# beehive-lab/GPULlama3.java

Hardware: AMD Instinct MI355X
Metric: tg128 tok/s (llama-bench), Llama-3-8B Q8_0 (higher is better)
Workload: dtype i8; 1 GPU; Llama-3-8B-random Q8_0 random-weight GGUF-layout model, tg128 at depth 0 (one step = 128 decode tokens, logits D2H inside the timed region); parallelism=single GPU, ranks=1, ctx=648

## Files before the change

### gpullama3.java_amd/csrc/gl3_api.hip

```cpp
#include <chrono>
#include <cstdio>
#include <cstdlib>
#include <cstring>
#include <vector>

#include "gl3_ctx.h"
#include "gl3_batch_plan.h"
#include "gl3_decode_kernels.h"
#include "gl3_rowlane_kernels.h"
#include "gl3_veclane_kernels.h"
#include "gl3_moe_kernels.h"
#include "gl3_kv_copy.h"

using namespace gl3;

static std::string g_create_err;

static double now_ms() {
    return std::chrono::duration<double, std::milli>(std::chrono::steady_clock::now().time_since_epoch()).count();
}


static size_t matvec_smem(int pro, int epi, const Q8Mat& w) {
    const int nm = epi == EPI_SWIGLU ? 2 : 1;
// ... 318 lines not shown
    if (!ctx->use_rccl) return GL3_OK;
    pr.begin(GL3_K_COLLECTIVE, 0);
    const int32_t r = gl3_all_gather(ctx, which, (size_t)count_per_rank);
    if (r != GL3_OK) return r;
    pr.end();
    return GL3_OK;
}

enum { ATT_LONG = 0, ATT_SHORT = 1, ATT_MID = 2 };
static int attn_mode(const gl3_ctx* ctx, int pos) {
    return (ctx->fused_attn_ok && pos < AF_MAXN) ? ATT_SHORT : pos < ctx->attn_mid ? ATT_MID : ATT_LONG;
}

static void launch_attention(gl3_ctx* ctx, int l, int which , int amode = ATT_LONG) {
    const gl3_model_desc& d = ctx->d;
    gl3_layer& L = ctx->layers[l];
    const size_t kv_layer = (size_t)d.ctx * ctx->kv_dim_l;
    const int kvmul = d.n_heads / d.n_kv_heads;
    AttnArgs aa{};
    aa.qkv = ctx->qkv; aa.kcache = ctx->kcache + l * kv_layer; aa.vcache = ctx->vcache + l * kv_layer;
    aa.rope_cr = ctx->rope_cr; aa.rope_ci = ctx->rope_ci; aa.qnorm = L.qnorm; aa.knorm = L.knorm; aa.bq = L.bq; aa.bk = L.bk; aa.bv = L.bv;
    aa.dyn = ctx->dyn_cur; aa.att = ctx->att; aa.xb = ctx->xb + (size_t)d.tp_rank * ctx->q_dim_l;
    aa.n_heads = ctx->heads_l; aa.n_kv_heads = ctx->kv_heads_l;
    aa.hs = d.head_size; aa.q_dim = ctx->q_dim_l; aa.kv_dim = ctx->kv_dim_l; aa.ctx = d.ctx;
    aa.eps = d.rms_eps; aa.arch = ctx->rope_arch; aa.att_mul = ctx->att_mul;
    const size_t sm1 = ((size_t)kvmul * d.head_size + (size_t)ATT_TT * (d.head_size + 4) + d.head_size) * 4;
    const int pv_rows = d.ctx < PV_ROWS ? d.ctx : PV_ROWS;
    aa.win = ctx->attn_win;
    aa.att_stride = (d.ctx + 3) & ~3;
    aa.att_t = ctx->att_t; aa.tmax = ctx->att_tmax; aa.sums = ctx->att_sums;
    aa.tp = tp_rec(ctx, l, TR_ATTN);
    const size_t sm2 = ((size_t)ctx->attn_win + (size_t)pv_rows * PV_COLS) * 4;
    if (which == 0 && amode == ATT_SHORT && ctx->fused_attn_ok) {
        attn_head_dispatch(d.head_size, [&](auto kern) { hipLaunchKernelGGL(kern, dim3(ctx->heads_l), dim3(256), attn_head_smem(d.head_size), ctx->stream, aa); });
        return;
    }
    static const bool scores_loop = env_flag("GL3_ATTN_SCORES_LOOP", true);
    if (which != 2 && amode == ATT_LONG && scores_loop && kvmul <= 4 && (d.head_size == 128 || d.head_size == 64)) {
        const dim3 sg(ctx->n_tsplit < SCL_WGS ? ctx->n_tsplit : SCL_WGS, ctx->kv_heads_l), sb(64 * (kvmul + SCL_LOADERS));
        const size_t sml = ((size_t)kvmul * d.head_size + 2 * (size_t)ATT_TT * (d.head_size + 4) + 2 * d.head_size) * 4;
        if (d.head_size == 128) hipLaunchKernelGGL(attn_scores_loop_kernel<128>, sg, sb, sml, ctx->stream, aa, ctx->n_tsplit);
        else hipLaunchKernelGGL(attn_scores_loop_kernel<64>, sg, sb, sml, ctx->stream, aa, ctx->n_tsplit);
    }
    else if (which != 2) hipLaunchKernelGGL(attn_scores_kernel, dim3(ctx->n_tsplit, ctx->kv_heads_l), dim3(64 * kvmul), sm1, ctx->stream, aa);
    if (which != 1 && amode == ATT_LONG) {
        const int exp_rows = (d.ctx + EXP_ROW - 1) / EXP_ROW;
        hipLaunchKernelGGL(attn_exp_kernel, dim3(exp_rows < EXP_GRID_MAX ? exp_rows : EXP_GRID_MAX, ctx->heads_l), dim3(256), 0, ctx->stream, aa, ctx->n_tsplit);
        hipLaunchKernelGGL(attn_sum_kernel, dim3(ctx->heads_l), dim3(256), attn_sum_smem(), ctx->stream, aa);
        hipLaunchKernelGGL(attn_pv_kernel, dim3(ctx->kv_heads_l * attn_pv_hq(kvmul) * (d.head_size / PV_COLS16)), dim3(64 * PV_WAVES), attn_pv_smem(), ctx->stream, aa);
    } else if (which != 1)
        hipLaunchKernelGGL(attn_softmax_pv_kernel, dim3(ctx->heads_l * (d.head_size / PV_COLS)), dim3(256), sm2, ctx->stream, aa);
}

static int32_t enqueue_decode(gl3_ctx* ctx, bool want_logits, gl3_kernel_times* kt, int amode) {
    const gl3_model_desc& d = ctx->d;
    hipStream_t s = ctx->stream;
    Prof pr{ctx, kt};
    const int rank = d.tp_rank;
    const bool q8 = ctx->emb.fmt == GL3_TYPE_Q8_0;
    int32_t r;
    Gl3Range step_range("gl3 decode step");

    pr.begin(GL3_K_OTHER, (uint64_t)d.dim / 32 * 34);
    const int fold = ctx->tp_fold, fmask = fold ? ctx->tp_fold_mask : 0, L_ = d.n_layers;
    uint32_t* vl_step = fold ? reinterpret_cast<uint32_t*>(ctx->arena.base + GL3_ARENA_STEP) : (uint32_t*)nullptr;
    if (ctx->emb.fmt == GL3_TYPE_Q8_0)
        hipLaunchKernelGGL(embed_q8t_kernel, dim3(1), dim3(256), 0, s, ctx->emb.w, ctx->emb.ng, d.dim, ctx->dyn_cur, ctx->x, ctx->emb_scale,
// ... 236 lines not shown
    const size_t kvn = ctx->kv_seq_stride * ctx->n_seqs;
    TRY(dmalloc(ctx, &ctx->kcache, kvn));
    TRY(dmalloc(ctx, &ctx->vcache, kvn + (size_t)PVT * ctx->kv_dim_l));
    TRYHIP(hipMemset(ctx->kcache, 0, kvn * 4));
    TRYHIP(hipMemset(ctx->vcache, 0, (kvn + (size_t)PVT * ctx->kv_dim_l) * 4));
    if (ctx->n_seqs > 1) TRY(dmalloc(ctx, &ctx->kv_copy_dst, ctx->n_seqs));
    TRY(dmalloc(ctx, &ctx->xn, d.dim));
    TRY(dmalloc(ctx, &ctx->qkv, ctx->q_dim_l + 2 * ctx->kv_dim_l));
    if (ctx->use_rccl) {
        if (tp > GL3_MAX_TP) return bail(GL3_E_UNSUPPORTED, "tp_size above 16");
        TRY(gl3_tp_arena_alloc(ctx));
        ctx->x = (float*)(ctx->arena.base + ctx->arena.off[GB_X]); ctx->xb = (float*)(ctx->arena.base + ctx->arena.off[GB_XB]);
        ctx->hb = (float*)(ctx->arena.base + ctx->arena.off[GB_HB]); ctx->logits = (float*)(ctx->arena.base + ctx->arena.off[GB_LOGITS]);
    } else {
        TRY(dmalloc(ctx, &ctx->x, d.dim));
        TRY(dmalloc(ctx, &ctx->xb, ctx->q_dim));
        TRY(dmalloc(ctx, &ctx->hb, d.hidden));
        TRY(dmalloc(ctx, &ctx->logits, d.vocab));
    }
    TRY(dmalloc(ctx, &ctx->att, (size_t)ctx->heads_l * ((d.ctx + 3) & ~3)));
    TRY(dmalloc(ctx, &ctx->att_t, attn_att_t_floats(ctx->kv_heads_l, d.n_heads / d.n_kv_heads, (d.ctx + 3) & ~3)));
    TRYHIP(hipMemset(ctx->att_t, 0, attn_att_t_floats(ctx->kv_heads_l, d.n_heads / d.n_kv_heads, (d.ctx + 3) & ~3) * 4));
    TRY(dmalloc(ctx, &ctx->att_tmax, (size_t)ctx->heads_l * ctx->n_tsplit));
    TRY(dmalloc(ctx, &ctx->att_sums, (size_t)ctx->heads_l));
    if (moe) TRY(moe_build_slots(ctx));
    TRYHIP((allow_big_lds<PRO_RMS, EPI_STORE>()));
    TRYHIP((allow_big_lds<PRO_QUANT, EPI_RESID>()));
    TRYHIP((allow_big_lds<PRO_RMS, EPI_SWIGLU>()));
    {
        ctx->fused_attn_ok = d.head_size % 4 == 0 && attn_head_smem(d.head_size) <= 150 * 1024 && !env_flag("GL3_NO_FUSED_ATTN", false);
        if (ctx->fused_attn_ok) {
            hipError_t ae = hipSuccess;
            attn_head_dispatch(d.head_size, [&](auto kern) { ae = hipFuncSetAttribute((const void*)kern, hipFuncAttributeMaxDynamicSharedMemorySize, 160 * 1024 - 256); });
            TRYHIP(ae);
        }
    }
    TRYHIP(hipFuncSetAttribute((const void*)matvec_q8t_kernel<PRO_QUANT, EPI_RESID, true, 8>, hipFuncAttributeMaxDynamicSharedMemorySize, 160 * 1024 - 256));
    TRYHIP(hipFuncSetAttribute((const void*)matvec_q8t_kernel<PRO_QUANT, EPI_RESID, true, 8, false, false, true>, hipFuncAttributeMaxDynamicSharedMemorySize, 160 * 1024 - 256));
    TRYHIP(hipFuncSetAttribute((const void*)matvec_q8t_kernel<PRO_QUANT, EPI_RESID, true, 8, false, true, true>, hipFuncAttributeMaxDynamicSharedMemorySize, 160 * 1024 - 256));
#define GL3_RL_LDS(...) TRYHIP(hipFuncSetAttribute((const void*)matvec_rl_kernel<__VA_ARGS__>, hipFuncAttributeMaxDynamicSharedMemorySize, 160 * 1024 - 256))
    GL3_RL_LDS(WT_F16, EPI_STORE); GL3_RL_LDS(WT_F16, EPI_RESID); GL3_RL_LDS(WT_F16, EPI_SWIGLU);
    GL3_RL_LDS(WT_Q4_0, EPI_STORE); GL3_RL_LDS(WT_Q4_0, EPI_RESID); GL3_RL_LDS(WT_Q4_0, EPI_SWIGLU);
#undef GL3_RL_LDS
    TRYHIP(hipFuncSetAttribute((const void*)rmsnorm_f32_kernel, hipFuncAttributeMaxDynamicSharedMemorySize, 160 * 1024 - 256));
    TRYHIP(hipFuncSetAttribute((const void*)attn_scores_kernel, hipFuncAttributeMaxDynamicSharedMemorySize, 128 * 1024));
    TRYHIP(hipFuncSetAttribute((const void*)attn_scores_loop_kernel<128>, hipFuncAttributeMaxDynamicSharedMemorySize, 128 * 1024));
    TRYHIP(hipFuncSetAttribute((const void*)attn_scores_loop_kernel<64>, hipFuncAttributeMaxDynamicSharedMemorySize, 128 * 1024));
    TRYHIP(hipFuncSetAttribute((const void*)attn_softmax_pv_kernel, hipFuncAttributeMaxDynamicSharedMemorySize, 150 * 1024));
    TRYHIP(hipFuncSetAttribute((const void*)attn_sum_kernel, hipFuncAttributeMaxDynamicSharedMemorySize, (int)attn_sum_smem()));
    TRYHIP(hipFuncSetAttribute((const void*)attn_pv_kernel, hipFuncAttributeMaxDynamicSharedMemorySize, (int)attn_pv_smem()));
    {
        const char* wv = getenv("GL3_ATTN_WINDOW");
        int wmax = wv && *wv ? atoi(wv) : 16384;
        if (wmax < PV_ROWS || wmax % PV_ROWS != 0 || wmax > 16384) return bail(GL3_E_ARG, "GL3_ATTN_WINDOW must be a multiple of 1024 between 1024 and 16384");
        ctx->attn_win = d.ctx <= wmax ? ((d.ctx + 3) & ~3) : wmax;
        const char* mv = getenv("GL3_ATTN_MID");
        ctx->attn_mid = mv && *mv ? atoi(mv) : 768;
    }
    TRY(dmalloc(ctx, &ctx->dyn, GL3_DYN_INTS));
    ctx->dyn_cur = ctx->dyn;
    TRY(dmalloc(ctx, &ctx->argmax, 2 + 2 * AMX_WGS));
    TRYHIP(hipMemset(ctx->argmax, 0, (2 + 2 * AMX_WGS) * sizeof(int)));
    if (d.flags & GL3_FLAG_LAYER_TAPS) TRY(dmalloc(ctx, &ctx->taps, (size_t)d.n_layers * d.dim));
    TRYHIP(hipHostMalloc((void**)&ctx->h_dyn, GL3_DYN_INTS * sizeof(int)));
    TRYHIP(hipHostMalloc((void**)&ctx->h_logits, (size_t)d.vocab * 4));
    TRYHIP(hipHostMalloc((void**)&ctx->h_argmax, sizeof(int)));
// ... 877 lines not shown
```

### gpullama3.java_amd/csrc/gl3_decode_kernels.h

```cpp
#pragma once
#include <hip/hip_runtime.h>
#include <stdint.h>

#include "gl3_seqsum.h"

namespace gl3 {

constexpr int TILE_BYTES = 2176;
constexpr int MV_AUX = 4;
__host__ __device__ constexpr int mv_threads(int npw) { return 64 * (npw + MV_AUX); }

enum { PRO_RMS = 0, PRO_QUANT = 1 };
enum { EPI_STORE = 0, EPI_RESID = 1, EPI_SWIGLU = 2 };
__host__ __device__ constexpr int mv_ch(int epi) { return epi == EPI_SWIGLU ? 4 : 8; }
__host__ __device__ constexpr int mv_seg_groups(int npw, int epi) { return npw * mv_ch(epi); }

typedef float v4f __attribute__((ext_vector_type(4)));

#ifdef GL3_MV_TIMING
__device__ long long gl3_mv_stamp[32];
#define ATT_STAMP(i) do { if (blockIdx.x == 0 && threadIdx.x == 0) gl3_mv_stamp[i] = wall_clock64(); } while (0)
#define MV_STAMP(i, cond) do { if (blockIdx.x == 0 && (cond)) gl3_mv_stamp[i] = clock64(); } while (0)
#define PV_T(...) __VA_ARGS__
constexpr int MV_WG_STAMPS = 1024;
__device__ unsigned long long gl3_mv_wg_stamp[MV_WG_STAMPS][8];
#define MV_WG_TIME(v) v = (unsigned long long)wall_clock64()
#define MV_WG_PUT(s, v, cond) do { if (blockIdx.x < MV_WG_STAMPS && blockIdx.y == 0 && (cond)) atomicMax(&gl3_mv_wg_stamp[blockIdx.x][s], v); } while (0)
#else
#define PV_T(...)
#define MV_STAMP(i, cond)
#define MV_WG_TIME(v)
#define MV_WG_PUT(s, v, cond)
#define ATT_STAMP(i)
#endif

constexpr int TPF_MAX_PEERS = 15;
struct TpWait {
    const uint32_t* flags;
    const uint32_t* step;
    uint32_t* err;
    int mul, add, tp, me;
    unsigned spin_limit;
};
struct TpPush {
    uint32_t* ticket;
    const uint32_t* step;
    int mul, add, npeers;
    long delta[TPF_MAX_PEERS];
    uint32_t* flag[TPF_MAX_PEERS];
};
struct TpRec { TpWait w; TpPush p; };

__device__ __forceinline__ void tp_wait(const TpWait& w) {
    const uint32_t need = (__hip_atomic_load(w.step, __ATOMIC_RELAXED, __HIP_MEMORY_SCOPE_AGENT) - 1u) * (uint32_t)w.mul + (uint32_t)w.add;
// ... 217 lines not shown
    if (t < 2) sync_w[t] = 0;

    if (wave < MV_PRODUCERS) {
        const int nt = (a.ng - wave + MV_PRODUCERS - 1) / MV_PRODUCERS;
        uint16_t sc[NM][CH];
        int4 lo[NM][CH], hi[NM][CH];
        auto issue = [&](int strip, int i0) {
#pragma unroll
            for (int u = 0; u < CH; ++u) {
                if (i0 + u < nt) {
                    const int g = wave + (i0 + u) * MV_PRODUCERS;
#pragma unroll
                    for (int m = 0; m < NM; ++m) {
                        const uint8_t* p = (m == 0 ? a.w : a.w2) + (size_t)strip * strip_bytes + (size_t)g * TILE_BYTES;
                        sc[m][u] = ld2<NT>(p + 2 * lane);
                        lo[m][u] = ld16<NT>(p + 128 + 16 * lane);
                        hi[m][u] = ld16<NT>(p + 1152 + 16 * lane);
                    }
                }
            }
        };
        auto compute = [&](int i0, float* pb) {
#pragma unroll
            for (int u = 0; u < CH; ++u) {
                if (i0 + u < nt) {
                    const int g = wave + (i0 + u) * MV_PRODUCERS;
                    const int xb = 4 * g + (lane >> 4);
                    const int4 xlo = *reinterpret_cast<const int4*>(xq + 32 * xb);
                    const int4 xhi = *reinterpret_cast<const int4*>(xq + 32 * xb + 16);
                    const float xsc = xs[xb];
#pragma unroll
                    for (int m = 0; m < NM; ++m) {
                        const int isum = dot32(lo[m][u], hi[m][u], xlo, xhi);
                        pb[(size_t)m * a.ng * 64 + g * 64 + lane] = (float)isum * (h2f(sc[m][u]) * xsc);
                    }
                }
            }
        };
        int strip = blockIdx.x;
        __syncthreads();
        if (strip < a.nstrips) issue(strip, 0);
        while (__hip_atomic_load(&sync_w[1], __ATOMIC_RELAXED, __HIP_MEMORY_SCOPE_WORKGROUP) == 0) __builtin_amdgcn_s_sleep(2);
        __builtin_amdgcn_fence(__ATOMIC_ACQUIRE, "workgroup");
        MV_STAMP(3, t == 0);
        int it = 0;
        for (; strip < a.nstrips; strip += gridDim.x, ++it) {
            float* pb = pbuf + (size_t)(it & 1) * NM * a.ng * 64;
            for (int i0 = 0; i0 < nt; i0 += CH) {
                if (it != 0 || i0 != 0) issue(strip, i0);
                compute(i0, pb);
                if (SEGS) {
                    MV_STAMP(4 + 2 * it, t == 0 && it < 4 && i0 + CH >= nt);
                    MV_WG_TIME(wg_t1);
                    lds_barrier();
                }
            }
            if (SEGS) {
                for (int b = (nt + CH - 1) / CH; b < nbatch; ++b) lds_barrier();
            } else {
                MV_STAMP(4 + 2 * it, t == 0 && it < 4);
                MV_WG_TIME(wg_t1);
                __syncthreads();
            }
            MV_STAMP(5 + 2 * it, t == 0 && it < 4);
        }
        MV_WG_PUT(0, wg_t0, t == 0); MV_WG_PUT(1, wg_t1, lane == 0);
        return;
// ... 53 lines not shown
        *reinterpret_cast<int4*>(xq + 32 * b) = z;
        *reinterpret_cast<int4*>(xq + 32 * b + 16) = z;
    }
    if (nquads <= NXV * 256) {
#pragma unroll
        for (int i = 0; i < NXV; ++i) {
            const int qd = ta + 256 * i;
            if (qd < nquads) {
                float4 v = xv[i];
                if (PRO == PRO_RMS) {
                    const float4 w = nwv[i];
                    v.x = w.x * (scale * v.x); v.y = w.y * (scale * v.y); v.z = w.z * (scale * v.z); v.w = w.w * (scale * v.w);
                }
                quantize_quad(v, qd, xq, xs);
            }
        }
    } else {
        for (int qd = ta; qd < nquads; qd += 256) {
            float4 v = *reinterpret_cast<const float4*>(a.x + 4 * qd);
            if (PRO == PRO_RMS) {
                const float4 w = *reinterpret_cast<const float4*>(a.norm_w + 4 * qd);
                v.x = w.x * (scale * v.x); v.y = w.y * (scale * v.y); v.z = w.z * (scale * v.z); v.w = w.w * (scale * v.w);
            }
            quantize_quad(v, qd, xq, xs);
        }
    }
    aux_sync();
    if (ta == 0) __hip_atomic_store(&sync_w[1], 1, __ATOMIC_RELEASE, __HIP_MEMORY_SCOPE_WORKGROUP);
    if (wave != MV_PRODUCERS) return;

    int it = 0;
    for (int strip = blockIdx.x; strip < a.nstrips; strip += gridDim.x, ++it) {
        const float* pb = pbuf + (size_t)(it & 1) * NM * a.ng * 64;
        v4f acc[NM];
#pragma unroll
        for (int m = 0; m < NM; ++m) acc[m] = (v4f){0.f, 0.f, 0.f, 0.f};
        for (int b = 0; b < nbatch; ++b) {
            if (SEGS) lds_barrier(); else __syncthreads();
            MV_STAMP(16 + 2 * it, lane == 0 && it < 4 && b == nbatch - 1);
            MV_WG_TIME(wg_t1);
            int g = b * SEG;
            const int ge = SEGS ? min(g + SEG, a.ng) : a.ng;
            for (; g + 8 <= ge; g += 8) {
                float av[NM][8];
#pragma unroll
                for (int m = 0; m < NM; ++m)
#pragma unroll
                    for (int u = 0; u < 8; ++u) av[m][u] = pb[(size_t)m * a.ng * 64 + (g + u) * 64 + lane];
#pragma unroll
                for (int u = 0; u < 8; ++u)
#pragma unroll
                    for (int m = 0; m < NM; ++m) acc[m] = __builtin_amdgcn_mfma_f32_16x16x4f32(av[m][u], 1.0f, acc[m], 0, 0, 0);
            }
            for (; g < ge; ++g)
#pragma unroll
                for (int m = 0; m < NM; ++m)
                    acc[m] = __builtin_amdgcn_mfma_f32_16x16x4f32(pb[(size_t)m * a.ng * 64 + g * 64 + lane], 1.0f, acc[m], 0, 0, 0);
        }
        MV_STAMP(17 + 2 * it, lane == 0 && it < 4);
        MV_WG_TIME(wg_t2);
        if ((lane & 15) < 4) {
            const int r = lane & 3;
            const int row = strip * 16 + 4 * (lane >> 4) + r;
            if (row < a.rows) {
                const float v0 = r == 0 ? acc[0][0] : r == 1 ? acc[0][1] : r == 2 ? acc[0][2] : acc[0][3];
                float res;
                if (EPI == EPI_STORE) res = v0 * a.out_scale;
                if (EPI == EPI_RESID) res = a.resid_in ? a.resid_in[row] + v0 * a.out_scale : v0 * a.out_scale;
                if (EPI == EPI_SWIGLU) {
                    const float v1 = r == 0 ? acc[NM - 1][0] : r == 1 ? acc[NM - 1][1] : r == 2 ? acc[NM - 1][2] : acc[NM - 1][3];
                    const float gte = v0 / (float)(1.0 + exp(-(double)v0));
                    res = gte * v1;
                }
                a.out[row] = res;
                if (TPF) tp_push_store(a.tp->p, a.out + row, res);
            }
        }
        PV_T(asm volatile("s_waitcnt vmcnt(0)" ::: "memory");)
        MV_WG_TIME(wg_t0);
        MV_WG_PUT(2, wg_t1, lane == 0); MV_WG_PUT(3, wg_t2, lane == 0); MV_WG_PUT(4, wg_t0, lane == 0);
    }
    if (TPF && a.tp->p.npeers) tp_publish(a.tp->p, gridDim.x);
}

static __global__ __launch_bounds__(256) void embed_q8t_kernel(const uint8_t* __restrict__ emb, int ng, int dim,
                                                         const int* __restrict__ dyn, float* __restrict__ x, float emb_scale,
                                                         const TpRec* tp = nullptr, uint32_t* step = nullptr) {
    if (step) {
        const uint32_t s = *step;
        __syncthreads();
        if (threadIdx.x == 0) *step = s + 1;
        if (tp) {
            TpWait w = tp->w;
            const uint32_t need = s * (uint32_t)w.mul;
            const int lane = threadIdx.x & 63;
            const bool mine = lane < w.tp && lane != w.me;
            unsigned spins = 0;
            for (;;) {
                const bool ok = !mine || (int32_t)(__hip_atomic_load(w.flags + (mine ? lane : 0), __ATOMIC_RELAXED, __HIP_MEMORY_SCOPE_SYSTEM) - need) >= 0;
                if (__builtin_amdgcn_ballot_w64(!ok) == 0) break;
                __builtin_amdgcn_s_sleep(8);
                if (++spins > w.spin_limit) { if (lane == 0) __hip_atomic_store(w.err, 1u, __ATOMIC_RELAXED, __HIP_MEMORY_SCOPE_SYSTEM); break; }
            }
// ... 25 lines not shown
    const float* bv;
    const int* dyn;
    float* att;
    float* xb;
    int n_heads, n_kv_heads, hs, q_dim, kv_dim, ctx;
    float eps;
    int arch;
    const int* seqv;
    const int* posv;
    size_t seq_stride;
    int qkv_stride, xb_stride;
    float att_mul;
    int win;
    int att_stride;
    float* att_t;
    float* tmax;
    float* sums;
    int group;
    uint8_t* xq_out; float* xs_out; int xq_slots;
    const TpRec* tp;
};

__device__ __forceinline__ void rope_head(float* v, int hs, const float* cr, const float* ci, int arch, int t0, int nthreads) {
    const int half = hs >> 1;
    for (int i = t0; i < half; i += nthreads) {
        const float fcr = cr[i], fci = ci[i];
        const int i0 = arch == 0 ? 2 * i : i, i1 = arch == 0 ? 2 * i + 1 : i + half;
        const float v0 = v[i0], v1 = v[i1];
        v[i0] = v0 * fcr - v1 * fci;
        v[i1] = v0 * fci + v1 * fcr;
    }
}

__device__ __forceinline__ void head_rmsnorm_wave(float* v, const float* __restrict__ w, int hs, float eps, int lane) {
    float ss = seq_sum_lds<true>(v, hs);
    ss /= (float)hs;
    ss += eps;
    ss = (float)(1.0 / sqrt((double)ss));
    for (int i = lane; i < hs; i += 64) v[i] = w[i] * (ss * v[i]);
}

constexpr int ATT_TT = 64;

static __global__ void attn_scores_kernel(const AttnArgs a) {
    extern __shared__ __attribute__((aligned(16))) float sm[];
    const int hs = a.hs, kvmul = a.n_heads / a.n_kv_heads, half = hs >> 1;
    float* q_s = sm;
    float* kt = q_s + kvmul * hs;
    float* cr_s = kt + ATT_TT * (hs + 4);
    float* ci_s = cr_s + half;
    const int t = threadIdx.x, nthr = blockDim.x;
    const int sp = blockIdx.x, kvh = blockIdx.y;
    const int pos = a.dyn[1];
    const int t0 = sp * ATT_TT;
    if (t0 > pos) return;
    const int t1 = min(pos + 1, t0 + ATT_TT);
    const bool owns_pos = (t1 == pos + 1);
    const int pitch = hs + 4;
    float* krow = kt + (pos - t0) * pitch;
    const int q4 = hs >> 2;
    const int nrows_cache = owns_pos ? (t1 - 1 - t0) : (t1 - t0);
    const int nk4 = nrows_cache * q4;
    constexpr int KMAX = 16;
    float4 kreg[KMAX];
    const int per = (nk4 + nthr - 1) / nthr;
#pragma unroll
    for (int u = 0; u < KMAX; ++u) {
        kreg[u] = make_float4(0.f, 0.f, 0.f, 0.f);
        if (u < per) {
            const int i = min(t + u * nthr, nk4 - 1);
            kreg[u] = *reinterpret_cast<const float4*>(a.kcache + (size_t)(t0 + i / q4) * a.kv_dim + kvh * hs + 4 * (i % q4));
// ... 166 lines not shown
#define SCL_USE(Q_, K_) do { _Pragma("unroll") for (int u = 0; u < 4; ++u) { \
            score = score + mul_f32_scalar(Q_[u].x, K_[u].x); score = score + mul_f32_scalar(Q_[u].y, K_[u].y); \
            score = score + mul_f32_scalar(Q_[u].z, K_[u].z); score = score + mul_f32_scalar(Q_[u].w, K_[u].w); } } while (0)
        SCL_RD(qa, ka, 0);
#pragma unroll
        for (int g = 0; g < HS / 16; g += 2) {
            SCL_RD(qb, kb, 4 * (g + 1));
            __builtin_amdgcn_sched_barrier(0);
            SCL_USE(qa, ka);
            __builtin_amdgcn_sched_barrier(0);
            if (g + 2 < HS / 16) SCL_RD(qa, ka, 4 * (g + 2));
            __builtin_amdgcn_sched_barrier(0);
            SCL_USE(qb, kb);
            __builtin_amdgcn_sched_barrier(0);
        }
#undef SCL_RD
#undef SCL_USE
        float my_score = -INFINITY;
        if (t0 + r < t1) {
            my_score = a.att_mul != 0.f ? score * a.att_mul : score / sqrt_hs;
            a.att[(size_t)(kvh * kvmul + hq) * a.att_stride + t0 + r] = my_score;
        }
        const float m = wave_max(my_score);
        if (r == 0) a.tmax[(size_t)(kvh * kvmul + hq) * n_tiles_max + sp] = m;
    }
    PV_T(if (blockIdx.x == 0 && blockIdx.y == 0 && t == 0) { gl3_mv_stamp[5] = cbw_; gl3_mv_stamp[6] = clock64() - cts_; gl3_mv_stamp[7] = cnt; })
}

constexpr int AF_MAXN = 128;
__host__ __device__ inline size_t attn_head_smem(int hs, int group = 1) {
    return ((size_t)group * hs + (size_t)AF_MAXN * (hs + 4) + (size_t)AF_MAXN * hs + (size_t)group * AF_MAXN + hs + 16) * 4;
}

template <int HS>
static __global__ __launch_bounds__(256, 1) void attn_head_kernel(const AttnArgs a) {
    extern __shared__ __attribute__((aligned(16))) float sm[];
    const int hs = HS > 0 ? HS : a.hs, kvmul = a.n_heads / a.n_kv_heads, half = hs >> 1, pitch = hs + 4, q4 = hs >> 2;
    const int q4sh = (q4 & (q4 - 1)) == 0 ? __ffs(q4) - 1 : -1;
    auto row_of = [&](int i) { return q4sh >= 0 ? i >> q4sh : i / q4; };
    auto col_of = [&](int i, int row) { return q4sh >= 0 ? i & (q4 - 1) : i - row * q4; };
    const int G = a.group > 1 ? a.group : 1;
    float* q_s = sm;
    float* kt = q_s + G * hs;
    float* vt = kt + AF_MAXN * pitch;
    float* e_s = vt + AF_MAXN * hs;
    float* cr_s = e_s + G * AF_MAXN;
    float* ci_s = cr_s + half;
    float* red = ci_s + half;
    const int t = threadIdx.x, lane = t & 63, wave = t >> 6;
    const int h0 = blockIdx.x * G, kvh = h0 / kvmul;
    const bool owner = (h0 % kvmul) == 0;
    const int bt = blockIdx.y;
    const int pos = a.seqv ? a.posv[bt] : a.dyn[1], n = pos + 1;
    const size_t kvoff = a.seqv ? (size_t)a.seqv[bt] * a.seq_stride : 0;
    const float* qkv = a.qkv + (size_t)bt * a.qkv_stride;
    float* kcache = a.kcache + kvoff;
    float* vcache = a.vcache + kvoff;
    ATT_STAMP(0);
    const int nk4 = pos * q4;
    constexpr int KMAX = 16;
    float4 kreg[KMAX], vreg[KMAX];
    const bool in_regs = nk4 <= KMAX * 256;
    const int per = in_regs ? (nk4 + 255) >> 8 : 0;
#pragma unroll
    for (int u = 0; u < KMAX; ++u) {
        kreg[u] = make_float4(0.f, 0.f, 0.f, 0.f);
        vreg[u] = make_float4(0.f, 0.f, 0.f, 0.f);
        if (u < per) {
            const int i = min(t + u * 256, nk4 - 1), ri = row_of(i);
            const size_t off = (size_t)ri * a.kv_dim + kvh * hs + 4 * col_of(i, ri);
            kreg[u] = *reinterpret_cast<const float4*>(kcache + off);
            vreg[u] = *reinterpret_cast<const float4*>(vcache + off);
        }
    }
    for (int i = t; i < G * hs; i += 256) q_s[i] = a.bq ? qkv[h0 * hs + i] + a.bq[h0 * hs + i] : qkv[h0 * hs + i];
    for (int i = t; i < half; i += 256) { cr_s[i] = a.rope_cr[(size_t)pos * half + i]; ci_s[i] = a.rope_ci[(size_t)pos * half + i]; }
    float* krow = kt + pos * pitch;
    for (int i = t; i < hs; i += 256) {
        krow[i] = a.bk ? qkv[a.q_dim + kvh * hs + i] + a.bk[kvh * hs + i] : qkv[a.q_dim + kvh * hs + i];
        vt[pos * hs + i] = a.bv ? qkv[a.q_dim + a.kv_dim + kvh * hs + i] + a.bv[kvh * hs + i] : qkv[a.q_dim + a.kv_dim + kvh * hs + i];
    }
    if (in_regs) {
#pragma unroll
        for (int u = 0; u < KMAX; ++u) {
            const int i = t + u * 256;
            if (i < nk4) {
                const int ri = row_of(i), ci = col_of(i, ri);
                *reinterpret_cast<float4*>(kt + ri * pitch + 4 * ci) = kreg[u];
                *reinterpret_cast<float4*>(vt + ri * hs + 4 * ci) = vreg[u];
            }
        }
    } else {
        for (int i = t; i < nk4; i += 256) {
            const int ri = row_of(i), ci = col_of(i, ri);
            const size_t off = (size_t)ri * a.kv_dim + kvh * hs + 4 * ci;
            *reinterpret_cast<float4*>(kt + ri * pitch + 4 * ci) = *reinterpret_cast<const float4*>(kcache + off);
            *reinterpret_cast<float4*>(vt + ri * hs + 4 * ci) = *reinterpret_cast<const float4*>(vcache + off);
        }
    }
    __syncthreads();
    ATT_STAMP(1);
    if (a.arch == 1) {
        for (int vec = wave; vec <= G; vec += 4)
            head_rmsnorm_wave(vec < G ? q_s + vec * hs : krow, vec < G ? a.qnorm : a.knorm, hs, a.eps, lane);
        __syncthreads();
    }
    for (int g = 0; g < G; ++g) rope_head(q_s + g * hs, hs, cr_s, ci_s, a.arch, t, 256);
    rope_head(krow, hs, cr_s, ci_s, a.arch, t, 256);
    __syncthreads();
    if (owner) {
        for (int i = t; i < hs; i += 256) {
            kcache[(size_t)pos * a.kv_dim + kvh * hs + i] = krow[i];
            vcache[(size_t)pos * a.kv_dim + kvh * hs + i] = vt[pos * hs + i];
        }
    }
    ATT_STAMP(2);
    const float sqrt_hs = (float)sqrt((double)hs);
    float sc = -INFINITY;
    for (int idx = t; idx < G * n; idx += 256) {
        const int g = idx / n, tt = idx - g * n;
        const float* q = q_s + g * hs;
        const float* kk = kt + tt * pitch;
        float score = 0.f;
        float4 qv = *reinterpret_cast<const float4*>(q), kv = *reinterpret_cast<const float4*>(kk);
        for (int j = 4; j < hs; j += 4) {
            const float4 qn = *reinterpret_cast<const float4*>(q + j), kn = *reinterpret_cast<const float4*>(kk + j);
            score = score + qv.x * kv.x; score = score + qv.y * kv.y; score = score + qv.z * kv.z; score = score + qv.w * kv.w;
            qv = qn; kv = kn;
        }
        score = score + qv.x * kv.x; score = score + qv.y * kv.y; score = score + qv.z * kv.z; score = score + qv.w * kv.w;
        sc = a.att_mul != 0.f ? score * a.att_mul : score / sqrt_hs;
        if (G > 1) e_s[g * AF_MAXN + tt] = sc;
    }
    ATT_STAMP(3);
    if (G == 1) {
        {
            const float wm = wave_max(t < n ? sc : -INFINITY);
            if (lane == 0) red[wave] = wm;
        }
        __syncthreads();
        const float mx = fmaxf(fmaxf(red[0], red[1]), fmaxf(red[2], red[3]));
        float ex = 0.f;
        if (t < n) { ex = (float)exp((double)(sc - mx)); e_s[t] = ex; }
        __syncthreads();
        ATT_STAMP(4);
        if (wave == 0) { const float sum = seq_sum_lds_ring(e_s, n); if (lane == 0) red[4] = sum; }
        __syncthreads();
        if (t < n) e_s[t] = ex / red[4];
        __syncthreads();
    } else {
        __syncthreads();
        for (int g = wave; g < G; g += 4) {
            float* e = e_s + g * AF_MAXN;
            const float s0 = lane < n ? e[lane] : -INFINITY, s1 = lane + 64 < n ? e[lane + 64] : -INFINITY;
            const float mx = wave_max(fmaxf(s0, s1));
            const float e0 = lane < n ? (float)exp((double)(s0 - mx)) : 0.f, e1 = lane + 64 < n ? (float)exp((double)(s1 - mx)) : 0.f;
            if (lane < n) e[lane] = e0;
            if (lane + 64 < n) e[lane + 64] = e1;
            __builtin_amdgcn_fence(__ATOMIC_RELEASE, "workgroup");
            __builtin_amdgcn_wave_barrier();
            __builtin_amdgcn_fence(__ATOMIC_ACQUIRE, "workgroup");
            const float sum = seq_sum_lds_ring(e, n);
            __builtin_amdgcn_wave_barrier();
            if (lane < n) e[lane] = e0 / sum;
            if (lane + 64 < n) e[lane + 64] = e1 / sum;
        }
        __syncthreads();
    }
    ATT_STAMP(5);
    for (int idx = t; idx < G * hs; idx += 256) {
        const int g = idx / hs, j = idx - g * hs;
        const float* e = e_s + g * AF_MAXN;
        const float* vj = vt + j;
        float acc = 0.f;
        int tt = 0;
        const int NG = n >> 2;
        if (NG >= 3) {
            float4 ea, eb, ec;
            float a0, a1, a2, a3, b0, b1, b2, b3, c0, c1, c2, c3;
#define PV_LD(G_, E_, V0_, V1_, V2_, V3_) do { const int r_ = 4 * min((G_), NG - 1); E_ = *reinterpret_cast<const float4*>(e + r_); \
            const float* vr_ = vj + r_ * hs; V0_ = vr_[0]; V1_ = vr_[hs]; V2_ = vr_[2 * hs]; V3_ = vr_[3 * hs]; } while (0)
#define PV_ACC(E_, V0_, V1_, V2_, V3_) do { acc = mul_f32_scalar(E_.x, V0_) + acc; acc = mul_f32_scalar(E_.y, V1_) + acc; \
            acc = mul_f32_scalar(E_.z, V2_) + acc; acc = mul_f32_scalar(E_.w, V3_) + acc; } while (0)
            PV_LD(0, ea, a0, a1, a2, a3); PV_LD(1, eb, b0, b1, b2, b3); PV_LD(2, ec, c0, c1, c2, c3);
            int gq = 0;
            for (; gq + 3 <= NG; gq += 3) {
                PV_ACC(ea, a0, a1, a2, a3); PV_LD(gq + 3, ea, a0, a1, a2, a3); __builtin_amdgcn_sched_barrier(0);
                PV_ACC(eb, b0, b1, b2, b3); PV_LD(gq + 4, eb, b0, b1, b2, b3); __builtin_amdgcn_sched_barrier(0);
                PV_ACC(ec, c0, c1, c2, c3); PV_LD(gq + 5, ec, c0, c1, c2, c3); __builtin_amdgcn_sched_barrier(0);
            }
            if (gq < NG) { PV_ACC(ea, a0, a1, a2, a3); ++gq; }
            if (gq < NG) { PV_ACC(eb, b0, b1, b2, b3); ++gq; }
#undef PV_ACC
#undef PV_LD
            tt = 4 * NG;
        }
        for (; tt < n; ++tt) acc = e[tt] * vj[tt * hs] + acc;
        if (a.xq_out) {
            float am = fabsf(acc);
            am = fmaxf(am, __builtin_bit_cast(float, __builtin_amdgcn_update_dpp(0, __builtin_bit_cast(int, am), 0xB1, 0xf, 0xf, false)));
            am = fmaxf(am, __builtin_bit_cast(float, __builtin_amdgcn_update_dpp(0, __builtin_bit_cast(int, am), 0x4E, 0xf, 0xf, false)));
            am = fmaxf(am, __builtin_bit_cast(float, __builtin_amdgcn_update_dpp(0, __builtin_bit_cast(int, am), 0x141, 0xf, 0xf, false)));
            am = fmaxf(am, __builtin_bit_cast(float, __builtin_amdgcn_update_dpp(0, __builtin_bit_cast(int, am), 0x140, 0xf, 0xf, false)));
            am = fmaxf(am, __shfl_xor(am, 16, 64));
            const float qs = am / 127.0f;
            const float ainv = qs != 0.f ? 1.0f / qs : 0.f;
            const float sv = acc * ainv;
            const int q0 = (int)(sv + copysignf(0.5f, sv)) & 0xFF;
            const int q1 = __builtin_amdgcn_update_dpp(0, q0, 0x55, 0xf, 0xf, false);
            const int q2 = __builtin_amdgcn_update_dpp(0, q0, 0xAA, 0xf, 0xf, false);
            const int q3 = __builtin_amdgcn_update_dpp(0, q0, 0xFF, 0xf, 0xf, false);
            const int el = (h0 + g) * hs + j;
            if ((lane & 3) == 0)
                *reinterpret_cast<uint32_t*>(a.xq_out + bdq_offset(el >> 2, bt, a.xq_slots)) = (uint32_t)q0 | ((uint32_t)q1 << 8) | ((uint32_t)q2 << 16) | ((uint32_t)q3 << 24);
            if ((lane & 31) == 0) a.xs_out[bds_offset(el >> 5, bt, a.xq_slots)] = (float)(_Float16)qs;
        } else {
            float* o = a.xb + (size_t)bt * a.xb_stride + (size_t)(h0 + g) * hs + j;
            *o = acc;
            if (a.tp) tp_push_store(a.tp->p, o, acc);
        }
    }
    ATT_STAMP(6);
    if (a.tp) tp_publish(a.tp->p, gridDim.x * gridDim.y * 4);
}

template <typename F>
static inline void attn_head_dispatch(int hs, F&& f) {
    if (hs == 128) f(attn_head_kernel<128>);
    else if (hs == 64) f(attn_head_kernel<64>);
    else f(attn_head_kernel<0>);
}

constexpr int PV_COLS = 16;
constexpr int PV_ROWS = 1024;

static __global__ __launch_bounds__(256) void attn_softmax_pv_kernel(const AttnArgs a) {
    extern __shared__ __attribute__((aligned(16))) float e_s[];
    const int hs = a.hs, kvmul = a.n_heads / a.n_kv_heads;
    const int nj = hs / PV_COLS;
    const int h = blockIdx.x / nj, j0 = (blockIdx.x % nj) * PV_COLS;
    const int t = threadIdx.x, lane = t & 63, wave = t >> 6, kvh = h / kvmul;
    const int n = a.dyn[1] + 1;
    float* vbuf = e_s + a.win;
    const float* vbase = a.vcache + kvh * hs + j0;
    constexpr int SU = PV_ROWS * 4 / 256;
    float4 sreg[SU];
#pragma unroll
    for (int u = 0; u < SU; ++u) sreg[u] = make_float4(0.f, 0.f, 0.f, 0.f);
    auto stage_issue = [&](int r0, int nr) {
#pragma unroll
        for (int u = 0; u < SU; ++u) {
            if (64 * u < nr) {
                const int row = min((t >> 2) + 64 * u, nr - 1);
                sreg[u] = *reinterpret_cast<const float4*>(vbase + (size_t)(r0 + row) * a.kv_dim + 4 * (t & 3));
            }
        }
    };
    auto stage_commit = [&](int nr) {
#pragma unroll
        for (int u = 0; u < SU; ++u)
            if ((t >> 2) + 64 * u < nr) *reinterpret_cast<float4*>(vbuf + 4 * (t + 256 * u)) = sreg[u];
    };
    __shared__ float red_s[8];
// ... 358 lines not shown
```

Baseline: 477.7 tok/s.

## Split fused short-context attention head kernel across value-column slices

The fused per-head attention kernel now launches a second grid dimension that splits the head's value columns into slices (2 for head size 128, 4 for 64). Each block recomputes the scores but loads and multiplies only its slice of V, so the decode attention stage gets more workgroups. The kernel also prefetches q/k/v/rope and norm weights into registers, defers V staging until after the softmax, and swaps some syncthreads for LDS-only barriers. The cost is redundant QK and softmax work in every slice, and the K-cache row is written only by slice zero.

```diff
diff --git a/gpullama3.java_amd/csrc/gl3_api.hip b/gpullama3.java_amd/csrc/gl3_api.hip
--- a/gpullama3.java_amd/csrc/gl3_api.hip
+++ b/gpullama3.java_amd/csrc/gl3_api.hip
@@ -374,7 +374,7 @@
     aa.tp = tp_rec(ctx, l, TR_ATTN);
     const size_t sm2 = ((size_t)ctx->attn_win + (size_t)pv_rows * PV_COLS) * 4;
     if (which == 0 && amode == ATT_SHORT && ctx->fused_attn_ok) {
-        attn_head_dispatch(d.head_size, [&](auto kern) { hipLaunchKernelGGL(kern, dim3(ctx->heads_l), dim3(256), attn_head_smem(d.head_size), ctx->stream, aa); });
+        attn_head_cs_dispatch(d.head_size, [&](auto kern, int cs, size_t smem) { hipLaunchKernelGGL(kern, dim3(ctx->heads_l, cs), dim3(256), smem, ctx->stream, aa); });
         return;
     }
     static const bool scores_loop = env_flag("GL3_ATTN_SCORES_LOOP", true);
@@ -677,6 +677,8 @@
         if (ctx->fused_attn_ok) {
             hipError_t ae = hipSuccess;
             attn_head_dispatch(d.head_size, [&](auto kern) { ae = hipFuncSetAttribute((const void*)kern, hipFuncAttributeMaxDynamicSharedMemorySize, 160 * 1024 - 256); });
+            TRYHIP(ae);
+            attn_head_cs_dispatch(d.head_size, [&](auto kern, int, size_t) { ae = hipFuncSetAttribute((const void*)kern, hipFuncAttributeMaxDynamicSharedMemorySize, 160 * 1024 - 256); });
             TRYHIP(ae);
         }
     }
diff --git a/gpullama3.java_amd/csrc/gl3_decode_kernels.h b/gpullama3.java_amd/csrc/gl3_decode_kernels.h
--- a/gpullama3.java_amd/csrc/gl3_decode_kernels.h
+++ b/gpullama3.java_amd/csrc/gl3_decode_kernels.h
@@ -19,7 +19,7 @@
 
 #ifdef GL3_MV_TIMING
 __device__ long long gl3_mv_stamp[32];
-#define ATT_STAMP(i) do { if (blockIdx.x == 0 && threadIdx.x == 0) gl3_mv_stamp[i] = wall_clock64(); } while (0)
+#define ATT_STAMP(i) do { if (blockIdx.x == 0 && blockIdx.y == 0 && threadIdx.x == 0) gl3_mv_stamp[i] = wall_clock64(); } while (0)
 #define MV_STAMP(i, cond) do { if (blockIdx.x == 0 && (cond)) gl3_mv_stamp[i] = clock64(); } while (0)
 #define PV_T(...) __VA_ARGS__
 constexpr int MV_WG_STAMPS = 1024;
@@ -551,11 +551,14 @@
     }
 }
 
-__device__ __forceinline__ void head_rmsnorm_wave(float* v, const float* __restrict__ w, int hs, float eps, int lane) {
+__device__ __forceinline__ float head_rms_scale(const float* v, int hs, float eps) {
     float ss = seq_sum_lds<true>(v, hs);
     ss /= (float)hs;
     ss += eps;
-    ss = (float)(1.0 / sqrt((double)ss));
+    return (float)(1.0 / sqrt((double)ss));
+}
+__device__ __forceinline__ void head_rmsnorm_wave(float* v, const float* __restrict__ w, int hs, float eps, int lane) {
+    const float ss = head_rms_scale(v, hs, eps);
     for (int i = lane; i < hs; i += 64) v[i] = w[i] * (ss * v[i]);
 }
 
@@ -788,87 +791,127 @@
     return ((size_t)group * hs + (size_t)AF_MAXN * (hs + 4) + (size_t)AF_MAXN * hs + (size_t)group * AF_MAXN + hs + 16) * 4;
 }
 
-template <int HS>
+__host__ __device__ inline size_t attn_head_cs_smem(int hs, int cs) {
+    return ((size_t)hs + (size_t)AF_MAXN * (hs + 4) + (size_t)AF_MAXN * (hs / cs) + (size_t)AF_MAXN + hs + 16) * 4;
+}
+
+template <int HS, int CS = 1>
 static __global__ __launch_bounds__(256, 1) void attn_head_kernel(const AttnArgs a) {
+    static_assert(CS == 1 || (HS > 0 && HS % (4 * CS) == 0), "a column slice is whole float4s of a compile-time head size");
     extern __shared__ __attribute__((aligned(16))) float sm[];
     const int hs = HS > 0 ? HS : a.hs, kvmul = a.n_heads / a.n_kv_heads, half = hs >> 1, pitch = hs + 4, q4 = hs >> 2;
-    const int q4sh = (q4 & (q4 - 1)) == 0 ? __ffs(q4) - 1 : -1;
-    auto row_of = [&](int i) { return q4sh >= 0 ? i >> q4sh : i / q4; };
-    auto col_of = [&](int i, int row) { return q4sh >= 0 ? i & (q4 - 1) : i - row * q4; };
-    const int G = a.group > 1 ? a.group : 1;
+    const int cw = hs / CS, c4 = cw >> 2;
+    auto row_of = [](int i, int w4) { return (w4 & (w4 - 1)) == 0 ? i >> (__ffs(w4) - 1) : i / w4; };
+    auto col_of = [](int i, int row, int w4) { return (w4 & (w4 - 1)) == 0 ? i & (w4 - 1) : i - row * w4; };
+    const int G = CS > 1 ? 1 : a.group > 1 ? a.group : 1;
     float* q_s = sm;
     float* kt = q_s + G * hs;
     float* vt = kt + AF_MAXN * pitch;
-    float* e_s = vt + AF_MAXN * hs;
+    float* e_s = vt + AF_MAXN * cw;
     float* cr_s = e_s + G * AF_MAXN;
     float* ci_s = cr_s + half;
     float* red = ci_s + half;
     const int t = threadIdx.x, lane = t & 63, wave = t >> 6;
     const int h0 = blockIdx.x * G, kvh = h0 / kvmul;
     const bool owner = (h0 % kvmul) == 0;
-    const int bt = blockIdx.y;
+    const int col0 = CS > 1 ? (int)blockIdx.y * cw : 0;
+    const int bt = CS > 1 ? 0 : blockIdx.y;
     const int pos = a.seqv ? a.posv[bt] : a.dyn[1], n = pos + 1;
     const size_t kvoff = a.seqv ? (size_t)a.seqv[bt] * a.seq_stride : 0;
     const float* qkv = a.qkv + (size_t)bt * a.qkv_stride;
     float* kcache = a.kcache + kvoff;
     float* vcache = a.vcache + kvoff;
     ATT_STAMP(0);
-    const int nk4 = pos * q4;
-    constexpr int KMAX = 16;
-    float4 kreg[KMAX], vreg[KMAX];
+    const int nk4 = pos * q4, nv4 = pos * c4;
+    constexpr int KMAX = HS > 0 ? (127 * (HS / 4) + 255) / 256 : 16, VMAX = HS > 0 ? (127 * (HS / CS / 4) + 255) / 256 : 16;
+    float4 kreg[KMAX], vreg[VMAX];
     const bool in_regs = nk4 <= KMAX * 256;
     const int per = in_regs ? (nk4 + 255) >> 8 : 0;
 #pragma unroll
     for (int u = 0; u < KMAX; ++u) {
         kreg[u] = make_float4(0.f, 0.f, 0.f, 0.f);
+        if (u < per) {
+            const int i = min(t + u * 256, nk4 - 1), ri = row_of(i, q4);
+            kreg[u] = *reinterpret_cast<const float4*>(kcache + (size_t)ri * a.kv_dim + kvh * hs + 4 * col_of(i, ri, q4));
+        }
+    }
+    const int nq = G * hs;
+    constexpr int QR = 4;
+    float qr[QR], k0 = 0.f, v0 = 0.f, cr0 = 0.f, ci0 = 0.f;
+#pragma unroll
+    for (int u = 0; u < QR; ++u) {
+        const int i = t + u * 256;
+        qr[u] = 0.f;
+        if (i < nq) qr[u] = a.bq ? qkv[h0 * hs + i] + a.bq[h0 * hs + i] : qkv[h0 * hs + i];
+    }
+    if (t < half) { cr0 = a.rope_cr[(size_t)pos * half + t]; ci0 = a.rope_ci[(size_t)pos * half + t]; }
+    if (t < hs) k0 = a.bk ? qkv[a.q_dim + kvh * hs + t] + a.bk[kvh * hs + t] : qkv[a.q_dim + kvh * hs + t];
+    if (t < cw) v0 = a.bv ? qkv[a.q_dim + a.kv_dim + kvh * hs + col0 + t] + a.bv[kvh * hs + col0 + t] : qkv[a.q_dim + a.kv_dim + kvh * hs + col0 + t];
+    constexpr int NWR = 4;
+    const bool nw_regs = a.arch == 1 && G == 1 && hs <= 64 * NWR;
+    float nw[NWR];
+#pragma unroll
+    for (int u = 0; u < NWR; ++u) {
+        nw[u] = 0.f;
+        if (nw_regs && wave < 2 && lane + 64 * u < hs) nw[u] = (wave ? a.knorm : a.qnorm)[lane + 64 * u];
+    }
+    float* krow = kt + pos * pitch;
+    for (int i = t + QR * 256; i < nq; i += 256) q_s[i] = a.bq ? qkv[h0 * hs + i] + a.bq[h0 * hs + i] : qkv[h0 * hs + i];
+    for (int i = t + 256; i < half; i += 256) { cr_s[i] = a.rope_cr[(size_t)pos * half + i]; ci_s[i] = a.rope_ci[(size_t)pos * half + i]; }
+    for (int i = t + 256; i < hs; i += 256) krow[i] = a.bk ? qkv[a.q_dim + kvh * hs + i] + a.bk[kvh * hs + i] : qkv[a.q_dim + kvh * hs + i];
+    for (int i = t + 256; i < cw; i += 256)
+        vt[pos * cw + i] = a.bv ? qkv[a.q_dim + a.kv_dim + kvh * hs + col0 + i] + a.bv[kvh * hs + col0 + i] : qkv[a.q_dim + a.kv_dim + kvh * hs + col0 + i];
+    __builtin_amdgcn_sched_barrier(0);
+#pragma unroll
+    for (int u = 0; u < VMAX; ++u) {
+        const int i = max(min(t + u * 256, nv4 - 1), 0), ri = row_of(i, c4);
         vreg[u] = make_float4(0.f, 0.f, 0.f, 0.f);
-        if (u < per) {
-            const int i = min(t + u * 256, nk4 - 1), ri = row_of(i);
-            const size_t off = (size_t)ri * a.kv_dim + kvh * hs + 4 * col_of(i, ri);
-            kreg[u] = *reinterpret_cast<const float4*>(kcache + off);
-            vreg[u] = *reinterpret_cast<const float4*>(vcache + off);
-        }
-    }
-    for (int i = t; i < G * hs; i += 256) q_s[i] = a.bq ? qkv[h0 * hs + i] + a.bq[h0 * hs + i] : qkv[h0 * hs + i];
-    for (int i = t; i < half; i += 256) { cr_s[i] = a.rope_cr[(size_t)pos * half + i]; ci_s[i] = a.rope_ci[(size_t)pos * half + i]; }
-    float* krow = kt + pos * pitch;
-    for (int i = t; i < hs; i += 256) {
-        krow[i] = a.bk ? qkv[a.q_dim + kvh * hs + i] + a.bk[kvh * hs + i] : qkv[a.q_dim + kvh * hs + i];
-        vt[pos * hs + i] = a.bv ? qkv[a.q_dim + a.kv_dim + kvh * hs + i] + a.bv[kvh * hs + i] : qkv[a.q_dim + a.kv_dim + kvh * hs + i];
-    }
+        vreg[u] = *reinterpret_cast<const float4*>(vcache + (size_t)ri * a.kv_dim + kvh * hs + col0 + 4 * col_of(i, ri, c4));
+    }
+    __builtin_amdgcn_sched_barrier(0);
+#pragma unroll
+    for (int u = 0; u < QR; ++u) { const int i = t + u * 256; if (i < nq) q_s[i] = qr[u]; }
+    if (t < half) { cr_s[t] = cr0; ci_s[t] = ci0; }
+    if (t < hs) krow[t] = k0;
+    if (t < cw) vt[pos * cw + t] = v0;
     if (in_regs) {
 #pragma unroll
         for (int u = 0; u < KMAX; ++u) {
             const int i = t + u * 256;
             if (i < nk4) {
-                const int ri = row_of(i), ci = col_of(i, ri);
+                const int ri = row_of(i, q4), ci = col_of(i, ri, q4);
                 *reinterpret_cast<float4*>(kt + ri * pitch + 4 * ci) = kreg[u];
-                *reinterpret_cast<float4*>(vt + ri * hs + 4 * ci) = vreg[u];
             }
         }
     } else {
         for (int i = t; i < nk4; i += 256) {
-            const int ri = row_of(i), ci = col_of(i, ri);
-            const size_t off = (size_t)ri * a.kv_dim + kvh * hs + 4 * ci;
-            *reinterpret_cast<float4*>(kt + ri * pitch + 4 * ci) = *reinterpret_cast<const float4*>(kcache + off);
-            *reinterpret_cast<float4*>(vt + ri * hs + 4 * ci) = *reinterpret_cast<const float4*>(vcache + off);
-        }
-    }
-    __syncthreads();
+            const int ri = row_of(i, q4), ci = col_of(i, ri, q4);
+            *reinterpret_cast<float4*>(kt + ri * pitch + 4 * ci) = *reinterpret_cast<const float4*>(kcache + (size_t)ri * a.kv_dim + kvh * hs + 4 * ci);
+        }
+    }
+    lds_barrier();
     ATT_STAMP(1);
     if (a.arch == 1) {
-        for (int vec = wave; vec <= G; vec += 4)
-            head_rmsnorm_wave(vec < G ? q_s + vec * hs : krow, vec < G ? a.qnorm : a.knorm, hs, a.eps, lane);
-        __syncthreads();
+        if (nw_regs) {
+            if (wave < 2) {
+                float* v = wave ? krow : q_s;
+                const float ss = head_rms_scale(v, hs, a.eps);
+#pragma unroll
+                for (int u = 0; u < NWR; ++u) { const int i = lane + 64 * u; if (i < hs) v[i] = nw[u] * (ss * v[i]); }
+            }
+        } else {
+            for (int vec = wave; vec <= G; vec += 4)
+                head_rmsnorm_wave(vec < G ? q_s + vec * hs : krow, vec < G ? a.qnorm : a.knorm, hs, a.eps, lane);
+        }
+        lds_barrier();
     }
     for (int g = 0; g < G; ++g) rope_head(q_s + g * hs, hs, cr_s, ci_s, a.arch, t, 256);
     rope_head(krow, hs, cr_s, ci_s, a.arch, t, 256);
-    __syncthreads();
+    lds_barrier();
     if (owner) {
-        for (int i = t; i < hs; i += 256) {
-            kcache[(size_t)pos * a.kv_dim + kvh * hs + i] = krow[i];
-            vcache[(size_t)pos * a.kv_dim + kvh * hs + i] = vt[pos * hs + i];
-        }
+        if (CS == 1 || blockIdx.y == 0)
+            for (int i = t; i < hs; i += 256) kcache[(size_t)pos * a.kv_dim + kvh * hs + i] = krow[i];
+        for (int i = t; i < cw; i += 256) vcache[(size_t)pos * a.kv_dim + kvh * hs + col0 + i] = vt[pos * cw + i];
     }
     ATT_STAMP(2);
     const float sqrt_hs = (float)sqrt((double)hs);
@@ -894,18 +937,17 @@
             const float wm = wave_max(t < n ? sc : -INFINITY);
             if (lane == 0) red[wave] = wm;
         }
-        __syncthreads();
+        lds_barrier();
         const float mx = fmaxf(fmaxf(red[0], red[1]), fmaxf(red[2], red[3]));
         float ex = 0.f;
         if (t < n) { ex = (float)exp((double)(sc - mx)); e_s[t] = ex; }
-        __syncthreads();
+        lds_barrier();
         ATT_STAMP(4);
         if (wave == 0) { const float sum = seq_sum_lds_ring(e_s, n); if (lane == 0) red[4] = sum; }
-        __syncthreads();
+        lds_barrier();
         if (t < n) e_s[t] = ex / red[4];
-        __syncthreads();
     } else {
-        __syncthreads();
+        lds_barrier();
         for (int g = wave; g < G; g += 4) {
             float* e = e_s + g * AF_MAXN;
             const float s0 = lane < n ? e[lane] : -INFINITY, s1 = lane + 64 < n ? e[lane + 64] : -INFINITY;
@@ -921,13 +963,28 @@
             if (lane < n) e[lane] = e0 / sum;
             if (lane + 64 < n) e[lane + 64] = e1 / sum;
         }
-        __syncthreads();
-    }
+    }
+    if (in_regs) {
+#pragma unroll
+        for (int u = 0; u < VMAX; ++u) {
+            const int i = t + u * 256;
+            if (i < nv4) {
+                const int ri = row_of(i, c4), ci = col_of(i, ri, c4);
+                *reinterpret_cast<float4*>(vt + ri * cw + 4 * ci) = vreg[u];
+            }
+        }
+    } else {
+        for (int i = t; i < nv4; i += 256) {
+            const int ri = row_of(i, c4), ci = col_of(i, ri, c4);
+            *reinterpret_cast<float4*>(vt + ri * cw + 4 * ci) = *reinterpret_cast<const float4*>(vcache + (size_t)ri * a.kv_dim + kvh * hs + col0 + 4 * ci);
+        }
+    }
+    __syncthreads();
     ATT_STAMP(5);
-    for (int idx = t; idx < G * hs; idx += 256) {
-        const int g = idx / hs, j = idx - g * hs;
+    for (int idx = t; idx < G * cw; idx += 256) {
+        const int g = idx / cw, jl = idx - g * cw, j = col0 + jl;
         const float* e = e_s + g * AF_MAXN;
-        const float* vj = vt + j;
+        const float* vj = vt + jl;
         float acc = 0.f;
         int tt = 0;
         const int NG = n >> 2;
@@ -935,7 +992,7 @@
             float4 ea, eb, ec;
             float a0, a1, a2, a3, b0, b1, b2, b3, c0, c1, c2, c3;
 #define PV_LD(G_, E_, V0_, V1_, V2_, V3_) do { const int r_ = 4 * min((G_), NG - 1); E_ = *reinterpret_cast<const float4*>(e + r_); \
-            const float* vr_ = vj + r_ * hs; V0_ = vr_[0]; V1_ = vr_[hs]; V2_ = vr_[2 * hs]; V3_ = vr_[3 * hs]; } while (0)
+            const float* vr_ = vj + r_ * cw; V0_ = vr_[0]; V1_ = vr_[cw]; V2_ = vr_[2 * cw]; V3_ = vr_[3 * cw]; } while (0)
 #define PV_ACC(E_, V0_, V1_, V2_, V3_) do { acc = mul_f32_scalar(E_.x, V0_) + acc; acc = mul_f32_scalar(E_.y, V1_) + acc; \
             acc = mul_f32_scalar(E_.z, V2_) + acc; acc = mul_f32_scalar(E_.w, V3_) + acc; } while (0)
             PV_LD(0, ea, a0, a1, a2, a3); PV_LD(1, eb, b0, b1, b2, b3); PV_LD(2, ec, c0, c1, c2, c3);
@@ -951,7 +1008,7 @@
 #undef PV_LD
             tt = 4 * NG;
         }
-        for (; tt < n; ++tt) acc = e[tt] * vj[tt * hs] + acc;
+        for (; tt < n; ++tt) acc = e[tt] * vj[tt * cw] + acc;
         if (a.xq_out) {
             float am = fabsf(acc);
             am = fmaxf(am, __builtin_bit_cast(float, __builtin_amdgcn_update_dpp(0, __builtin_bit_cast(int, am), 0xB1, 0xf, 0xf, false)));
@@ -985,6 +1042,13 @@
     if (hs == 128) f(attn_head_kernel<128>);
     else if (hs == 64) f(attn_head_kernel<64>);
     else f(attn_head_kernel<0>);
+}
+constexpr int AF_CS128 = 2, AF_CS64 = 4;
+template <typename F>
+static inline void attn_head_cs_dispatch(int hs, F&& f) {
+    if (hs == 128) f(attn_head_kernel<128, AF_CS128>, AF_CS128, attn_head_cs_smem(128, AF_CS128));
+    else if (hs == 64) f(attn_head_kernel<64, AF_CS64>, AF_CS64, attn_head_cs_smem(64, AF_CS64));
+    else f(attn_head_kernel<0>, 1, attn_head_smem(hs));
 }
 
 constexpr int PV_COLS = 16;
```

New measurement: 482.4 tok/s (median of 6 runs). Within noise of the previous version (+1.0%).

## Replace MFMA partial-sum reduction with transposed LDS layout and scalar adds

Applied to the files above, without the earlier changes.

Producers now write each group's partial products in a transposed LDS layout, so that one lane's four consecutive floats belong to the same output row. The single reducer wave then sums its row with float4 LDS reads and inline-asm v_add_f32 chains, software-pipelined across three register buffers and pinned with sched_barrier. This replaces the MFMA-based reduction with a fixed add order, and SwiGLU fetches its second matrix's sum with a shuffle. The aim is to cut reducer latency on the critical path, at the cost of only 16*NM lanes doing work and a serial dependent add chain.

```diff
diff --git a/gpullama3.java_amd/csrc/gl3_decode_kernels.h b/gpullama3.java_amd/csrc/gl3_decode_kernels.h
--- a/gpullama3.java_amd/csrc/gl3_decode_kernels.h
+++ b/gpullama3.java_amd/csrc/gl3_decode_kernels.h
@@ -303,7 +303,7 @@
 #pragma unroll
                     for (int m = 0; m < NM; ++m) {
                         const int isum = dot32(lo[m][u], hi[m][u], xlo, xhi);
-                        pb[(size_t)m * a.ng * 64 + g * 64 + lane] = (float)isum * (h2f(sc[m][u]) * xsc);
+                        pb[(size_t)m * a.ng * 64 + g * 64 + 4 * (lane & 15) + (lane >> 4)] = (float)isum * (h2f(sc[m][u]) * xsc);
                     }
                 }
             }
@@ -423,43 +423,68 @@
     int it = 0;
     for (int strip = blockIdx.x; strip < a.nstrips; strip += gridDim.x, ++it) {
         const float* pb = pbuf + (size_t)(it & 1) * NM * a.ng * 64;
-        v4f acc[NM];
-#pragma unroll
-        for (int m = 0; m < NM; ++m) acc[m] = (v4f){0.f, 0.f, 0.f, 0.f};
+        const float* p = pb + (size_t)(lane >> 4) * a.ng * 64 + 4 * (lane & 15);
+        float acc = 0.f;
         for (int b = 0; b < nbatch; ++b) {
             if (SEGS) lds_barrier(); else __syncthreads();
             MV_STAMP(16 + 2 * it, lane == 0 && it < 4 && b == nbatch - 1);
             MV_WG_TIME(wg_t1);
             int g = b * SEG;
             const int ge = SEGS ? min(g + SEG, a.ng) : a.ng;
-            for (; g + 8 <= ge; g += 8) {
-                float av[NM][8];
-#pragma unroll
-                for (int m = 0; m < NM; ++m)
-#pragma unroll
-                    for (int u = 0; u < 8; ++u) av[m][u] = pb[(size_t)m * a.ng * 64 + (g + u) * 64 + lane];
-#pragma unroll
-                for (int u = 0; u < 8; ++u)
-#pragma unroll
-                    for (int m = 0; m < NM; ++m) acc[m] = __builtin_amdgcn_mfma_f32_16x16x4f32(av[m][u], 1.0f, acc[m], 0, 0, 0);
-            }
-            for (; g < ge; ++g)
-#pragma unroll
-                for (int m = 0; m < NM; ++m)
-                    acc[m] = __builtin_amdgcn_mfma_f32_16x16x4f32(pb[(size_t)m * a.ng * 64 + g * 64 + lane], 1.0f, acc[m], 0, 0, 0);
+            if (lane < 16 * NM) {
+                constexpr int UG = 4;
+                float4 ra[4], rb[4], rc[4];
+#define MV_RDU(R_, U_) do { const float* q_ = p + (g + (U_) * UG) * 64; _Pragma("unroll") for (int j = 0; j < 4; ++j) \
+                    R_[j] = *reinterpret_cast<const float4*>(q_ + j * 64); } while (0)
+#define MV_ADDU(R_) asm volatile( \
+                    "v_add_f32 %0, %1, %0\n\tv_add_f32 %0, %2, %0\n\tv_add_f32 %0, %3, %0\n\tv_add_f32 %0, %4, %0\n\t" \
+                    "v_add_f32 %0, %5, %0\n\tv_add_f32 %0, %6, %0\n\tv_add_f32 %0, %7, %0\n\tv_add_f32 %0, %8, %0\n\t" \
+                    "v_add_f32 %0, %9, %0\n\tv_add_f32 %0, %10, %0\n\tv_add_f32 %0, %11, %0\n\tv_add_f32 %0, %12, %0\n\t" \
+                    "v_add_f32 %0, %13, %0\n\tv_add_f32 %0, %14, %0\n\tv_add_f32 %0, %15, %0\n\tv_add_f32 %0, %16, %0" \
+                    : "+v"(acc) : "v"(R_[0].x), "v"(R_[0].y), "v"(R_[0].z), "v"(R_[0].w), "v"(R_[1].x), "v"(R_[1].y), "v"(R_[1].z), "v"(R_[1].w), \
+                                  "v"(R_[2].x), "v"(R_[2].y), "v"(R_[2].z), "v"(R_[2].w), "v"(R_[3].x), "v"(R_[3].y), "v"(R_[3].z), "v"(R_[3].w))
+#define MV_PIN() __builtin_amdgcn_sched_barrier(0)
+                const int nu = (ge - g) / UG;
+                int u = 0;
+                if (nu >= 3) {
+                    MV_RDU(ra, 0); MV_RDU(rb, 1); MV_RDU(rc, 2); MV_PIN();
+                    for (; u + 6 <= nu; u += 3) {
+                        MV_ADDU(ra); MV_PIN(); MV_RDU(ra, u + 3); MV_PIN();
+                        MV_ADDU(rb); MV_PIN(); MV_RDU(rb, u + 4); MV_PIN();
+                        MV_ADDU(rc); MV_PIN(); MV_RDU(rc, u + 5); MV_PIN();
+                    }
+                    const int rem = nu - u - 3;
+                    MV_ADDU(ra); MV_PIN();
+                    if (rem == 0) {
+                        MV_ADDU(rb); MV_PIN(); MV_ADDU(rc);
+                    } else if (rem == 1) {
+                        MV_RDU(ra, u + 3); MV_PIN(); MV_ADDU(rb); MV_PIN(); MV_ADDU(rc); MV_PIN(); MV_ADDU(ra);
+                    } else {
+                        MV_RDU(ra, u + 3); MV_PIN(); MV_ADDU(rb); MV_PIN(); MV_RDU(rb, u + 4); MV_PIN(); MV_ADDU(rc); MV_PIN(); MV_ADDU(ra); MV_PIN(); MV_ADDU(rb);
+                    }
+                    u = nu;
+                }
+                for (; u < nu; ++u) { MV_RDU(ra, u); MV_ADDU(ra); }
+#undef MV_PIN
+#undef MV_ADDU
+#undef MV_RDU
+                for (g += nu * UG; g < ge; ++g) {
+                    const float4 q = *reinterpret_cast<const float4*>(p + g * 64);
+                    acc = acc + q.x; acc = acc + q.y; acc = acc + q.z; acc = acc + q.w;
+                }
+            }
         }
         MV_STAMP(17 + 2 * it, lane == 0 && it < 4);
         MV_WG_TIME(wg_t2);
-        if ((lane & 15) < 4) {
-            const int r = lane & 3;
-            const int row = strip * 16 + 4 * (lane >> 4) + r;
+        const float v1 = EPI == EPI_SWIGLU ? __shfl_down(acc, 16, 64) : 0.f;
+        if (lane < 16) {
+            const int row = strip * 16 + lane;
             if (row < a.rows) {
-                const float v0 = r == 0 ? acc[0][0] : r == 1 ? acc[0][1] : r == 2 ? acc[0][2] : acc[0][3];
+                const float v0 = acc;
                 float res;
                 if (EPI == EPI_STORE) res = v0 * a.out_scale;
                 if (EPI == EPI_RESID) res = a.resid_in ? a.resid_in[row] + v0 * a.out_scale : v0 * a.out_scale;
                 if (EPI == EPI_SWIGLU) {
-                    const float v1 = r == 0 ? acc[NM - 1][0] : r == 1 ? acc[NM - 1][1] : r == 2 ? acc[NM - 1][2] : acc[NM - 1][3];
                     const float gte = v0 / (float)(1.0 + exp(-(double)v0));
                     res = gte * v1;
                 }
```

Result: no change. 477.2 tok/s before, 475.3 tok/s after (-0.4%).
